# gabo99cas/minimal_volumetric_path_tracer

Hardware: AMD Instinct MI355X
Metric: Msamples/s (pixels×spp/s) at 1024²; per-channel RMSE vs CPU PPM (higher is better)
Workload: dtype f64; 1 GPU; ff 1024x1024x256spp default scene, sigma_a 0.001 sigma_s 0.009; width=1024, height=1024, spp=256, estimator=ff, parallelism=1 GPU, inflight=3

## Files before the change

minimal_volumetric_path_tracer_amd/csrc/vpt_device.h:

```cpp
#ifndef VPT_DEVICE_H
#define VPT_DEVICE_H

#include <hip/hip_runtime.h>
#include <stdint.h>

#include "vpt_math.h"
#include "vpt_rng.h"
#include "vpt_scene.h"

#define VPT_DEV __device__ static inline __attribute__((always_inline))
#define VPT_PI 3.14159265358979323846
#define VPT_MAXFLOAT ((double)3.40282346638528859812e+38F)
#define VPT_DBL_MAX 1.7976931348623157e+308
#ifndef VPT_ISECT_UNROLL
#define VPT_ISECT_UNROLL 5
#endif
#ifndef VPT_DECIDE_GROUP
#define VPT_DECIDE_GROUP 5
#endif
static_assert(VPT_DECIDE_GROUP >= 1, "spheres are taken G >= 1 at a time");

namespace vpt {

#define VPT_UNLIKELY(c) __builtin_expect(!!(c), 0)
#define VPT_LIKELY(c) __builtin_expect(!!(c), 1)

#define ISECT_SQRT(x) vm_sqrt(x)
#ifndef VPT_ISECT_CLASS
#define VPT_ISECT_CLASS 1
#endif

#ifndef VPT_SECTIONS
#define VPT_SECTIONS 0
#endif
enum {
    SECT_SCHED = 0, SECT_LOAD, SECT_S_PLIGHT, SECT_S_MIS, SECT_S_MIS_ISECT, SECT_S_BDSF, SECT_M_SS, SECT_M_SS_DIR,
    SECT_M_SS_ISECT, SECT_M_SS_SHADOW, SECT_M_PHASE, SECT_CONT, SECT_A_PREP, SECT_A_DECIDE, SECT_A_ISECT, SECT_STORE,
    SECT_S_TOTAL, SECT_M_TOTAL, SECT_A_CAMERA, SECT_A_DECIDE_IN, SECT_M_SHADOW_IN, SECT_A_CAMERA_IN, SECT_M_EQA,
    SECT_M_TR, SECT_A_UNIT, SECT_A_R2, SECT_USED,
    SECT_N = 32
};
#if VPT_SECTIONS
static __device__ unsigned long long g_vpt_sect[3 * SECT_N];
__device__ static inline __attribute__((always_inline)) uint32_t* sect_lds()
{
    __shared__ uint32_t a[8][3 * SECT_USED];
    return &a[(threadIdx.x >> 6) & 7][0];
}
#endif
__device__ static inline __attribute__((always_inline)) uint32_t sect_now()
{
#if VPT_SECTIONS
    return (uint32_t)__builtin_amdgcn_s_memtime();
#else
    return 0;
#endif
}
__device__ static inline __attribute__((always_inline)) void sect_add(int k, uint32_t t0)
{
#if VPT_SECTIONS
    const uint32_t dt = sect_now() - t0;
    const unsigned long long act = (unsigned long long)__ballot(1);
    const int first = __ffsll(act) - 1;
    if ((int)(threadIdx.x & 63) == first) {
        uint32_t* a = sect_lds();
        a[k] += dt;
        a[SECT_USED + k] += 1;
        a[2 * SECT_USED + k] += (uint32_t)__popcll(act);
    }
#else
    (void)k;
    (void)t0;
#endif
}
__device__ static inline __attribute__((always_inline)) void sect_init()
{
#if VPT_SECTIONS
    for (int l = threadIdx.x & 63; l < 3 * SECT_USED; l += 64) sect_lds()[l] = 0;
#endif
}
__device__ static inline __attribute__((always_inline)) void sect_flush()
{
#if VPT_SECTIONS
    for (int l = threadIdx.x & 63; l < 3 * SECT_USED; l += 64) {
        const uint32_t v = sect_lds()[l];
        atomicAdd(&g_vpt_sect[l < SECT_USED ? l : l < 2 * SECT_USED ? SECT_N + l - SECT_USED : 2 * SECT_N + l - 2 * SECT_USED],
                  (unsigned long long)v);
    }
#endif
}
#define SECT_BEGIN(name) const uint32_t _sect_##name = sect_now()
#define SECT_END(name, k) sect_add(k, _sect_##name)
// ... 99 lines not shown
            tmin = tact;
            id = i;
        }
    }
}

#ifndef VPT_TAKE_IN
#define VPT_TAKE_IN 1
#endif
#ifndef VPT_ISECT_ZERO
#define VPT_ISECT_ZERO 1
#endif
template <bool ZR = false>
VPT_DEV void sphere_test(double b, double det, int i, double& tmin, int& id, contact_t& contact)
{
    if (!VPT_TAKE_IN) {
        sphere_take(sphere_tact(b, det), i, tmin, id, contact);
        return;
    }
    if (det >= 0) {
        const double sq = (VPT_ISECT_ZERO && ZR) ? vm_sqrt_isect_z(det) : VPT_ISECT_CLASS ? vm_sqrt_isect(det) : ISECT_SQRT(det);
        const double t2 = -b + sq;
        const double t1 = -b - sq;
        sphere_take(t1 < 0.0001 ? t2 : t1, i, tmin, id, contact);
    }
}

template <bool COUNT, bool ZR = false>
VPT_DEV int scene_intersect(const DevScene* __restrict__ S, Sampler<COUNT>& smp, dv3 o, dv3 d, double& t,
                            int& id, bool skip3)
{
    double tmin = VPT_DBL_MAX;
    contact_t contact = 0;
    const int n = S->n;
#pragma unroll VPT_ISECT_UNROLL
    for (int i = 0; i < n; ++i) {
        const GeoSphere g = S->geo[i];
        if (skip3 && g.mat3) continue;
        double ocx = o.x - g.px, ocy = o.y - g.py, ocz = o.z - g.pz;
        double b = ocx * d.x + ocy * d.y + ocz * d.z;
        double cc = ocx * ocx + ocy * ocy + ocz * ocz;
        double det = b * b - cc + g.r2;
        sphere_test<ZR>(b, det, i, tmin, id, contact);
    }
    smp.tests(skip3 ? S->n_non3 : n);
    if (contact) {
        t = tmin;
        return 1;
    }
    t = 0;
    return 0;
}

template <int G, bool COUNT, bool ZR = false>
VPT_DEV int scene_intersect_grouped(const DevScene* __restrict__ S, Sampler<COUNT>& smp, dv3 o, dv3 d, double& t,
                                    int& id)
{
    static_assert(G >= 1, "spheres are taken G >= 1 at a time");
    double tmin = VPT_DBL_MAX;
    contact_t contact = 0;
    const int n = S->n;
    int i = 0;
    for (; i + G <= n; i += G) {
        double b[G], det[G];
#pragma unroll
        for (int k = 0; k < G; ++k) {
            const GeoSphere g = S->geo[i + k];
            const double ocx = o.x - g.px, ocy = o.y - g.py, ocz = o.z - g.pz;
            b[k] = ocx * d.x + ocy * d.y + ocz * d.z;
            const double cc = ocx * ocx + ocy * ocy + ocz * ocz;
            det[k] = b[k] * b[k] - cc + g.r2;
        }
#pragma unroll
        for (int k = 0; k < G; ++k) {
            sphere_test<ZR>(b[k], det[k], i + k, tmin, id, contact);
        }
    }
    for (; i < n; ++i) {
        const GeoSphere g = S->geo[i];
        const double ocx = o.x - g.px, ocy = o.y - g.py, ocz = o.z - g.pz;
        const double b = ocx * d.x + ocy * d.y + ocz * d.z;
        const double cc = ocx * ocx + ocy * ocy + ocz * ocz;
        const double det = b * b - cc + g.r2;
        sphere_test<ZR>(b, det, i, tmin, id, contact);
    }
    smp.tests(n);
    if (contact) {
        t = tmin;
        return 1;
    }
    t = 0;
    return 0;
}

template <int G, bool COUNT, bool ZR = false>
VPT_DEV int scene_intersect_grouped_oc(const DevScene* __restrict__ S, Sampler<COUNT>& smp, const double (*oc)[4],
                                       dv3 d, double& t, int& id)
{
    static_assert(G >= 1, "spheres are taken G >= 1 at a time");
    double tmin = VPT_DBL_MAX;
    contact_t contact = 0;
    const int n = S->n;
    int i = 0;
    for (; i + G <= n; i += G) {
        double b[G], det[G];
#pragma unroll
        for (int k = 0; k < G; ++k) {
            const double ocx = oc[i + k][0], ocy = oc[i + k][1], ocz = oc[i + k][2], cc = oc[i + k][3];
            b[k] = ocx * d.x + ocy * d.y + ocz * d.z;
            det[k] = b[k] * b[k] - cc + S->geo[i + k].r2;
        }
#pragma unroll
        for (int k = 0; k < G; ++k) sphere_test<ZR>(b[k], det[k], i + k, tmin, id, contact);
    }
    for (; i < n; ++i) {
        const double ocx = oc[i][0], ocy = oc[i][1], ocz = oc[i][2], cc = oc[i][3];
        const double b = ocx * d.x + ocy * d.y + ocz * d.z;
        const double det = b * b - cc + S->geo[i].r2;
        sphere_test<ZR>(b, det, i, tmin, id, contact);
    }
    smp.tests(n);
    if (contact) {
        t = tmin;
        return 1;
// ... 1066 lines not shown
    double dist;
    double pdf;
    int id;
    int src;
};

enum { EV_END = 0, EV_SURF = 1, EV_MED = 2 };

VPT_DEV void vpt_opaque(Path& p)
{
    vpt_opaque(p.o);
    vpt_opaque(p.d);
    vpt_opaque(p.beta);
    vpt_opaque(p.L);
    vpt_opaque(p.depth);
}
VPT_DEV void vpt_sink(const Path& p)
{
    vpt_sink(p.o);
    vpt_sink(p.d);
    vpt_sink(p.beta);
    vpt_sink(p.L);
    vpt_sink(p.depth);
}
VPT_DEV void vpt_opaque(Event& e)
{
    vpt_opaque(e.t);
    vpt_opaque(e.dist);
    vpt_opaque(e.pdf);
    vpt_opaque(e.id);
    vpt_opaque(e.src);
}
VPT_DEV void vpt_sink(const Event& e)
{
    vpt_sink(e.t);
    vpt_sink(e.dist);
    vpt_sink(e.pdf);
    vpt_sink(e.id);
    vpt_sink(e.src);
}

template <bool COUNT>
VPT_DEV bool continue_path(Sampler<COUNT>& smp, const Path& p, const Medium& m)
{
    if (m.max_depth > 0 && p.depth >= m.max_depth) return false;
    if (COUNT) smp.cnt.iterations++;
    const double q = 1 - 0.6;
    return !(smp.next() < q);
}

template <int EST>
VPT_DEV constexpr bool est_free_flight() { return EST == 0 || EST == 2 || EST == 3; }

template <int EST, bool COUNT>
VPT_DEV int decide(const DevScene* __restrict__ S, Sampler<COUNT>& smp, Path& p, Event& e, const Medium& m)
{
    const double sigma_t = m.sigma_a + m.sigma_s;
    int id = 0;
    double t = 0.0;
    SECT_BEGIN(di);
#if VPT_DUP == DUP_DECIDE_ISECT
    {
        dv3 o2 = p.o, d2 = p.d;
        vpt_opaque(o2);
        vpt_opaque(d2);
        double t2 = 0;
        int id2 = 0;
        const int h2 = scene_intersect_grouped<VPT_DECIDE_GROUP>(S, smp, o2, d2, t2, id2);
        vpt_sink(t2);
        vpt_sink(id2);
        vpt_sink(h2);
    }
#endif
    const bool hit = scene_intersect_grouped<VPT_DECIDE_GROUP>(S, smp, p.o, p.d, t, id);
    SECT_END(di, SECT_A_ISECT);
    if constexpr (EST == 5) {
        if (COUNT) smp.cnt.iterations++;
        e.t = t;
        e.id = id;
        e.src = 0;
        if (!hit) return EV_END;
        if (S->sph[id].radiance[0] > 0) {
            if (p.depth < 1) p.L = sph_rad(S, id);
            return EV_END;
        }
        return EV_SURF;
    }
    if (!hit) t = VPT_MAXFLOAT;
    e.t = t;
    e.id = id;
    if (EST == 3) {
        const double TrActual = hit ? transmitance(p.o, add(p.o, scl(p.d, t)), sigma_t) : 0.0;
        e.src = 0;
        e.dist = -lm_log(1 - smp.next()) / sigma_t;
        e.pdf = (sigma_t * lm_exp(sigma_t * e.dist * -1.0)) * (1.0 - TrActual);
        if (!(e.dist > t)) return EV_MED;
        if (sph_flag(S->m_emitter, id)) {
            p.L = add(p.L, mul(p.beta, sph_rad(S, id)));
            return EV_END;
        }
        return EV_SURF;
    }
    const int count = S->n_emit;
    if (VPT_UNLIKELY(count == 0)) return EV_END;
    e.src = emit_pick(S, (int)(smp.next() * count), count);
    bool surf;
    if (est_free_flight<EST>()) {
        e.dist = -lm_log(1 - smp.next()) / sigma_t;
        surf = e.dist > t;
    } else {
        const double psurf = EST == 1 ? lm_exp(sigma_t * t * -1.0)
                                      : (hit ? transmitance(p.o, add(p.o, scl(p.d, t)), sigma_t) : 0.0);
        (void)smp.next();
        e.pdf = psurf;
        surf = EST == 1 ? smp.next() < psurf : smp.next() <= psurf;
    }
    if (!surf) return EV_MED;
    if (sph_flag(S->m_emitter, id)) {
        if (p.depth == 0) p.L = EST == 0 ? mul(sph_rad(S, id), p.beta) : sph_rad(S, id);
        return EV_END;
    }
    return EV_SURF;
}

template <int EST, bool COUNT, int MK = -1, int PT = -1>
VPT_DEV void surface_event(const DevScene* __restrict__ S, Sampler<COUNT>& smp, Path& p, const Event& e,
                           const Medium& m, bool cont = true, int lk = -1)
{
    const int ptk = PT >= 0 ? PT : lk;
    const double sigma_t = m.sigma_a + m.sigma_s;
    const double continueprob = 0.6;
    const int id = e.id, src = e.src;
    const dv3 xs = add(p.o, scl(p.d, e.t));
    const dv3 nx = nrm(sub(xs, sph_p(S, id)));
    if (EST == 3) {
        dv3 wi = mk(0, 0, 0);
        double pdf = 0;
        dv3 fs = bdsf<COUNT, MK>(S, smp, wi, p.d, nx, pdf, id);
        wi = nrm(wi);
        const double cosine = dot(nx, wi);
        p.beta = scl(scl(scl(mul(p.beta, fs), (1 / continueprob)), cosine), (1 / pdf));
        p.o = xs;
        p.d = wi;
        p.depth++;
        return;
    }
    const double probSource = 1.0 / S->n_emit;
    const double alpha = S->sph[id].alpha;
    SECT_BEGIN(pl);
    dv3 Ldp = mk(0, 0, 0);
    bool plight_zero = false;
    if (ptk == 0 && S->n_mat3 == 0) {
        const dv3 lx = sub(sph_p(S, src), xs);
        const double dd = dot(lx, lx);
        const double distance = vm_sqrt(dd);
        const bool fin = dd > 0 && dd < VPT_DBL_MAX && nx.x - nx.x == 0 && nx.y - nx.y == 0 && nx.z - nx.z == 0;
        const bool zero = S->sph[src].r > 0.0001 && !(distance < S->sph[src].r) && fin;
        plight_zero = __ballot(!zero) == 0;
        if (plight_zero) smp.tests(2 * S->n);
    }
    Frame Fn = {};
    if (MK == 0 && VPT_FRAME_CSE) Fn = make_frame(nx);
#if VPT_DUP == DUP_PLIGHT
    if (!plight_zero) {
        dv3 xs2 = xs, nx2 = nx, d2 = p.d;
        int id2 = id, src2 = src;
        double a2 = alpha;
        Frame F2 = Fn;
        vpt_opaque(xs2);
        vpt_opaque(nx2);
        vpt_opaque(d2);
// ... 532 lines not shown
```

minimal_volumetric_path_tracer_amd/csrc/vpt_glibm.h:

```cpp
#ifndef VPT_GLIBM_H
#define VPT_GLIBM_H

#if defined(__HIPCC__)
#define GM_TABLE(name, n) __device__ static const double name[n]
#else
#define GM_TABLE(name, n) static const double name[n]
#endif
#include "vpt_glibm_tables.h"

#define GM_UNLIKELY(c) __builtin_expect(!!(c), 0)

VM_QUAL int32_t gm_hi(double x) { return (int32_t)(vm_as_u64(x) >> 32); }
VM_QUAL uint32_t gm_lo(double x) { return (uint32_t)vm_as_u64(x); }
VM_QUAL double gm_fma(double a, double b, double c) { return fma(a, b, c); }
VM_QUAL double gm_fnma(double a, double b, double c) { return fma(-a, b, c); }

VM_TABLE(gm_sc_tab, {
    -0x1.addffc2fcdf59p-26, 0x1.71de27b9a7ed9p-19, -0x1.a01a019db08b8p-13, 0x1.1111111110ecep-7,
    -0x1.5555555555555p-3,
    0x1.11110e829872fp-7, -0x1.5555555555515p-3,
    0x1.6c16bedd9e239p-10, -0x1.5555555555535p-5,
    0x1.8p+45,
    0x1.45f306dc9c883p-1, 0x1.8p52,
    0x1.921fb58000000p+0, -0x1.dde973c000000p-27,
// ... 228 lines not shown
    const double r = gm_fnma(t * t, z, 1.0);
    double q;
    VM_HORNER_T(q, K + GA_RT3, 4, r);
    t = q * t;
    const double c = z * t;
    const double h = gm_fnma(t * 0.5, c, 1.5);
    const double t27 = VM_T(K, GA_T27);
    const double y = gm_fnma(t27, c, gm_fma(c, t27, c));
    const double cc = gm_fnma(y, y, z) / gm_fma(h, c, y);
    double p;
    VM_HORNER_T(p, K + GA_F6, 6, z);
    const double pr = (p * z) * (y + cc);
    const double s = (cc + pr) + y;
    return x == 1.0 ? 0.0 : s + s;
}

VM_TABLE(gm_exp_tab, {
    0x1.71547652b82fep7, 0x1.8p52, -0x1.62e42fefa0000p-8, -0x1.cf79abc9e3b3ap-47,
    0x1.ffffffffffdbdp-2, 0x1.555555555543cp-3, 0x1.55555cf172b91p-5, 0x1.1111167a4d017p-7})
VM_TABLE(gm_log_tab, {
    -0x1.ffffffffffdcbp-3, 0x1.5555555555577p-2, 0x1.24924a344de3p-3, -0x1.55555556745a7p-3,
    -0x1.999eb43b068ffp-4, 0x1.c7184282ad6cap-4, 0x1.999999995dd0cp-3, -0x1.fffffa4423d65p-4,
    0x1.78182f7afd085p-4, -0x1.5521375d145cdp-4, 0x1p27,
    0x1.62e42fefa3800p-1, 0x1.ef35793c76730p-45, -0x1.fffffffeb4590p-3, 0x1.555555551305bp-2,
    -0x1.55575e506c89fp-3, 0x1.999b324f10111p-3, -0x1.0000000000001p-1})
enum { GE_INVLN2N = 0, GE_SHIFT, GE_NLN2HI, GE_NLN2LO, GE_C2, GE_C3, GE_C4, GE_C5 };
enum { GL_B0 = 0, GL_TWO27 = 10, GL_LN2HI, GL_LN2LO, GL_A0, GL_A1, GL_A2, GL_A3, GL_AH };

#define GM_EXP_T(i) gl_tab[(0xAF9D0ull - GL_TAB_LO) / 8 + (i)]
#define GM_LOG_T(i) gl_tab[(0xB0270ull - GL_TAB_LO) / 8 + (i)]

VM_QUAL double gm_exp(double x)
{
    vm_ct* K = vm_tab(gm_exp_tab);
    const uint32_t abstop = (uint32_t)(vm_as_u64(x) >> 52) & 0x7ffu;
    const double z = gm_fma(x, VM_T(K, GE_INVLN2N), VM_T(K, GE_SHIFT));
    const uint64_t ki = vm_as_u64(z);
    const double kd = z - VM_T(K, GE_SHIFT);
    double r = gm_fma(kd, VM_T(K, GE_NLN2HI), x);
    r = gm_fma(kd, VM_T(K, GE_NLN2LO), r);
    const uint32_t idx = 2u * (uint32_t)(ki & 0x7fu);
    const double tail = vm_as_f64(GM_EXP_T(idx));
    const uint64_t sbits = GM_EXP_T(idx + 1) + (ki << 45);
    const double r2 = r * r;
    const double p23 = gm_fma(r, VM_T(K, GE_C3), VM_T(K, GE_C2));
    const double p45 = gm_fma(r, VM_T(K, GE_C5), VM_T(K, GE_C4));
    const double tmp = gm_fma(r2 * r2, p45, gm_fma(p23, r2, r + tail));
    const double scale = vm_as_f64(sbits);
    double v = gm_fma(scale, tmp, scale);
    VM_RARE_FIX(abstop - 0x3c9u >= 0x3fu, v, gl_exp(x));
    return v;
}

VM_QUAL double gm_log(double x)
{
    vm_ct* K = vm_tab(gm_log_tab);
    const uint64_t ix = vm_as_u64(x);
    const uint32_t top = (uint32_t)(ix >> 48);
    const double r1 = x - 1.0;
    const double rr = r1 * r1;
    const double r3 = r1 * rr;
    double a = gm_fma(r1, VM_T(K, GL_B0), VM_T(K, GL_B0 + 1));
    double b = gm_fma(r1, VM_T(K, GL_B0 + 2), VM_T(K, GL_B0 + 3));
    double c = gm_fma(r1, VM_T(K, GL_B0 + 4), VM_T(K, GL_B0 + 5));
    a = gm_fma(rr, VM_T(K, GL_B0 + 6), a);
    b = gm_fma(rr, VM_T(K, GL_B0 + 7), b);
    c = gm_fma(rr, VM_T(K, GL_B0 + 8), c);
    c = gm_fma(r3, VM_T(K, GL_B0 + 9), c);
    c = gm_fma(c, r3, b);
    c = gm_fma(c, r3, a);
    const double two27 = VM_T(K, GL_TWO27);
    const double rhi = gm_fnma(two27, r1, gm_fma(r1, two27, r1));
    const double rhi2 = rhi * rhi;
    const double ah = -0.5;
    const double hi1 = gm_fma(rhi2, ah, r1);
    double lo1 = gm_fma(rhi2, ah, r1 - hi1);
    lo1 = gm_fma(ah * (r1 - rhi), r1 + rhi, lo1);
    double v1 = hi1 + gm_fma(c, r3, lo1);
    v1 = ix == 0x3ff0000000000000ull ? 0.0 : v1;
    const uint64_t tmp = ix + 0xc01a000000000000ull;
    const uint32_t i = (uint32_t)(tmp >> 45) & 0x7fu;
    const int k = (int)((int64_t)tmp >> 52);
    const double zz = vm_as_f64(ix - (tmp & 0xfff0000000000000ull));
    const double kd = (double)k;
    const double invc = vm_as_f64(GM_LOG_T(2 * i)), logc = vm_as_f64(GM_LOG_T(2 * i + 1));
    const double r = gm_fma(zz, invc, -1.0);
    const double w = gm_fma(kd, VM_T(K, GL_LN2HI), logc);
    const double hi = r + w;
    const double r2 = r * r;
    double lo = gm_fma(kd, VM_T(K, GL_LN2LO), (w - hi) + r);
    lo = gm_fma(r2, VM_T(K, GL_AH), lo);
    double q = gm_fma(r, VM_T(K, GL_A2), VM_T(K, GL_A3));
    q = gm_fma(q, r2, gm_fma(r, VM_T(K, GL_A0), VM_T(K, GL_A1)));
    const double v2 = gm_fma(r * r2, q, lo) + hi;
    double v = ix + 0xc012000000000000ull <= 0x308ffffffffffull ? v1 : v2;
    VM_RARE_FIX(top - 0x0010u >= 0x7ff0u - 0x0010u, v, gl_log(x));
    return v;
}

VM_TABLE(gm_atan2_tab, {
    0x1.375f08b31cbcep-4, -0x1.7458022b13c25p-4, 0x1.c71c6e5129a3bp-4, -0x1.24924923f7603p-3,
    0x1.99999999997fdp-3, -0x1.5555555555555p-2,
    0x1.921fb54442d18p+0, 0x1.1a62633145c07p-54,
    0x1p-500, 0x1p500, 0x1p52})
enum { GT_D13 = 0, GT_HPI = 6, GT_HPI1, GT_TM500, GT_T500, GT_TWO52 };
#define GM_CIJ(i, j) vm_as_f64(gl_tab[(0xBE0E0ull - GL_TAB_LO) / 8 + 7 * (i) + (j)])

VM_QUAL double gm_atan2(double y, double x)
{
    vm_ct* K = vm_tab(gm_atan2_tab);
    const double ax = vm_fabs(x), ay = vm_fabs(y);
    const int de = (int)((uint32_t)gm_hi(y) & 0x7ff00000u) - (int)((uint32_t)gm_hi(x) & 0x7ff00000u);
    const int ci = ax > ay;
    const double num = ci ? ay : ax, den = ci ? ax : ay;
    const double u = num / den;
    const double v5 = den * u;
    const double v7 = gm_fma(den, u, -v5);
    const double du = ((num - v5) - v7) / den;
    const double v = u * u;
    double p;
    VM_HORNER_T(p, K + GT_D13, 6, v);
    const double uv = u * v;
    const double hpi = VM_T(K, GT_HPI), hpi1 = VM_T(K, GT_HPI1);
    const double z_i_poly = u + gm_fma(uv, p, du);
    const double t2 = hpi - u;
    const double z_ii_poly = ((((hpi - t2) - u) + hpi1) - du) - uv * p + t2;
    int i = (int)(gm_fma(u, 256.0, VM_T(K, GT_TWO52)) - VM_T(K, GT_TWO52)) - 16;
    i = i < 0 ? 0 : i > 240 ? 240 : i;
    const double c0 = GM_CIJ(i, 0), c1 = GM_CIJ(i, 1), c2 = GM_CIJ(i, 2), c3 = GM_CIJ(i, 3);
    const double c4 = GM_CIJ(i, 4), c5 = GM_CIJ(i, 5), c6 = GM_CIJ(i, 6);
    const double t3 = u - c0;
    const double w = du + t3;
    const double dw = vm_fabs(t3) > vm_fabs(du) ? (t3 - w) + du : (du - w) + t3;
    double q = gm_fma(w, c6, c5);
    q = gm_fma(w, q, c4);
    q = gm_fma(w, q, c3);
    const double z_i_tab = gm_fma(w, c2, gm_fma(dw, c2, (w * w) * q)) + c1;
    const double w2 = t3 + du;
    double q2 = gm_fma(w2, c6, c5);
    q2 = gm_fma(w2, q2, c4);
    q2 = gm_fma(w2, q2, c3);
    q2 = gm_fma(w2, q2, c2);
    const double z_ii_tab = (hpi - c1) + gm_fnma(w2, q2, hpi1);
    const int small = u < 0.0625;
    const double z = ci ? (small ? z_i_poly : z_i_tab) : (small ? z_ii_poly : z_ii_tab);
    double r = vm_copysign(de > 0x38fffff ? hpi : z, y);
    const double tm500 = VM_T(K, GT_TM500), t500 = VM_T(K, GT_T500);
    const int rare = !(x > 0.0) || !(ay > 0.0) || !(x < __builtin_inf()) || !(ay < __builtin_inf()) ||
                     de < -0x38fffff || ax < tm500 || ay < tm500 || ax > t500 || ay > t500;
    VM_RARE_FIX(rare, r, gl_atan2(y, x));
    return r;
// ... 139 lines not shown
```

minimal_volumetric_path_tracer_amd/csrc/vpt_host.cpp:

```cpp
#include <math.h>
#include <stdarg.h>
#include <stdio.h>
#include <stdlib.h>
#include <string.h>

#include <string>
#include <vector>

#include <thread>

#include "vpt_accum.h"
#include "vpt_grid.h"
#include "vpt_internal.h"
#include "vpt_rng.h"

static thread_local std::string g_err;

int vpt_fail(int code, const char* fmt, ...)
{
    char buf[512];
    va_list ap;
    va_start(ap, fmt);
    vsnprintf(buf, sizeof buf, fmt, ap);
    va_end(ap);
    g_err = buf;
    return code;
}

void vpt_clear_error(void) { g_err.clear(); }

int vpt_int_grid_check(const vpt_grid_desc* desc, const float* density, const char* who)
{
    if (!desc || !density) return vpt_fail(VPT_E_INVALID, "%s: NULL grid", who);
    const int32_t n[3] = {desc->nx, desc->ny, desc->nz};
    switch (vpt_grid_bad(n, desc->lo, desc->hi, density)) {
    case 1: return vpt_fail(VPT_E_INVALID, "%s: grid %d x %d x %d (each dimension >= 1, at most 2^27 voxels)", who,
                            desc->nx, desc->ny, desc->nz);
    case 2: return vpt_fail(VPT_E_INVALID, "%s: the box must be finite with hi > lo", who);
    case 3: return vpt_fail(VPT_E_INVALID, "%s: densities must be finite and >= 0", who);
    }
    return VPT_OK;
}

extern "C" {

const char* vpt_last_error(void) { return g_err.c_str(); }
int vpt_abi_version(void) { return VPT_ABI_VERSION; }

uint64_t vpt_stream_state(uint64_t seed, uint64_t pixel_idx, uint64_t sample)
{
    return vpt_stream_start(seed, pixel_idx, sample);
}

void vpt_default_params(vpt_params* p)
{
    if (!p) return;
    memset(p, 0, sizeof *p);
    p->width = 1024;
    p->height = 768;
    p->spp = 16;
    p->fb_format = VPT_FB_F32;
    p->medium.sigma_a = 0.001;
    p->medium.sigma_s = 0.009;
    p->medium.hg_g = 0.0;
    p->medium.max_depth = 0;
    p->medium.estimator = VPT_FREE_FLIGHT;
    p->medium.march_step = 0.1;
    p->medium.march_light = 7;
    p->seed = 0x5EED0001ull;
    double dx = 0, dy = -0.042612, dz = -1;
    double inv = 1.0 / sqrt(dx * dx + dy * dy + dz * dz);
    p->camera.o[0] = 0; p->camera.o[1] = 11.2; p->camera.o[2] = 214;
    p->camera.d[0] = dx * inv; p->camera.d[1] = dy * inv; p->camera.d[2] = dz * inv;
    p->fov_scale = 0.5095;
    p->band_rows = p->height;
    p->band_stride = 1;
    p->band_offset = 0;
}

static void set_sphere(vpt_sphere* s, double r, double px, double py, double pz, double cr, double cg, double cb,
                       double lr, double lg, double lb, int mat, const double* eta, const double* kappa, double alpha)
{
    memset(s, 0, sizeof *s);
    s->r = r;
    s->p[0] = px; s->p[1] = py; s->p[2] = pz;
    s->c[0] = cr; s->c[1] = cg; s->c[2] = cb;
    s->radiance[0] = lr; s->radiance[1] = lg; s->radiance[2] = lb;
    s->material = mat;
    if (eta) memcpy(s->eta, eta, sizeof s->eta);
    if (kappa) memcpy(s->kappa, kappa, sizeof s->kappa);
    s->alpha = alpha;
}

int vpt_default_scene(vpt_sphere* out, int cap)
{
    vpt_sphere s[10];
    static const double al_eta[3] = {1.66058, 0.88143, 0.521467};
// ... 239 lines not shown
```

minimal_volumetric_path_tracer_amd/csrc/vpt_internal.h:

```cpp
#ifndef VPT_INTERNAL_H
#define VPT_INTERNAL_H

#include "../../include/vpt.h"

int vpt_fail(int code, const char* fmt, ...);
void vpt_clear_error(void);

int vpt_int_device(const vpt_context* ctx);
const unsigned* vpt_int_guard_flag(const vpt_context* ctx);
int vpt_int_check_guard(vpt_context* ctx, const char* who);
int vpt_int_check_params(const vpt_context* ctx, const vpt_params* p);
int vpt_int_pool_pass(vpt_context* ctx, const vpt_params* p, int C, int k0, int k1, const unsigned* d_tiles,
                      unsigned n_tiles, double* d_partials, unsigned* d_queue);

int vpt_int_grid_check(const vpt_grid_desc* desc, const float* density, const char* who);

#endif
```

minimal_volumetric_path_tracer_amd/csrc/vpt_kernels.hip:

```cpp
#include <hip/hip_runtime.h>

#include <math.h>
#include <stdlib.h>
#include <string.h>

#include <memory>
#include <mutex>
#include <vector>

#include "vpt_device.h"
#include "vpt_pool.h"
#include "vpt_wave.h"
#include "vpt_internal.h"

#ifndef VPT_MIS_TU
#define VPT_MIS_TU 1
#endif
#if VPT_MIS_TU
namespace vpt {
extern template __global__ void pool_kernel<1, false>(PoolParams P0, Medium m0, const DevScene* __restrict__ S,
                                                      unsigned long long* counters, unsigned long long* stats);
extern template __global__ void pool_kernel<1, false, true>(PoolParams P0, Medium m0, const DevScene* __restrict__ S,
                                                            unsigned long long* counters, unsigned long long* stats);
}
// ... 73 lines not shown
    x_new[3 * i + 1] = xn.y;
    x_new[3 * i + 2] = xn.z;
    idsource[i] = id;
    out_states[i] = smp.X;
}

__global__ void math_probe_kernel(int fn, const double* x, const double* y, double* out, int n)
{
    int i = blockIdx.x * blockDim.x + threadIdx.x;
    if (i >= n) return;
    double a = x[i], b = y[i], r = 0;
    switch (fn) {
    case 0: r = vm_sqrt(a); break;
    case 1: r = lm_exp(a); break;
    case 2: r = lm_log(a); break;
    case 3: r = lm_sin(a); break;
    case 4: r = lm_cos(a); break;
    case 5: r = lm_tan(a); break;
    case 6: r = lm_atan(a); break;
    case 7: r = lm_acos(a); break;
    case 8: r = lm_atan2(a, b); break;
    case 12: r = vm_inv_sqrt(a); break;
    case 10:
    case 11: {
        double sv, cv;
        lm_sincos_acos(a, &sv, &cv);
        r = fn == 10 ? sv : cv;
        break;
    }
    case 14:
    case 15:
    case 16:
    case 17: {
        double q[4];
        lm_dir_trig(a, b, &q[0], &q[1], &q[2], &q[3]);
        r = q[fn - 14];
        break;
    }
    case 18: {
        double bb = b;
        __asm__ volatile("" : "+v"(bb));
        r = vm_div_by(a, vm_rcp_of(bb));
        break;
    }
    case 19: r = hemi_cosine_prob(a); break;
    case 20: {
        double inv, q;
        inv_and_ratio(a, b, inv, q);
        r = __longlong_as_double(__double_as_longlong(inv) ^ __double_as_longlong(q));
        break;
    }
    case 21: r = vm_sqrt_isect(a); break;
    case 22: r = vm_sqrt_isect_z(a); break;
    default: r = a / b; break;
    }
    out[i] = r;
}

__global__ void phase_probe_kernel(double g, double dx, double dy, double dz, const uint64_t* X, int n, double* dirs,
                                   uint64_t* Xout, const double* wl, int nw, double* vals)
{
    const int i = blockIdx.x * blockDim.x + threadIdx.x;
    const dv3 din = mk(dx, dy, dz);
    if (i < n) {
        Sampler<false> smp;
        smp.X = X[i];
        smp.g = g;
        smp.cnt.tests = smp.cnt.iterations = smp.cnt.draw_mismatch = 0;
        const dv3 w = phase_sample(smp, din);
        dirs[3 * i] = w.x;
        dirs[3 * i + 1] = w.y;
        dirs[3 * i + 2] = w.z;
        Xout[i] = smp.X;
    }
    if (i < nw) vals[i] = phase_value(g, din, mk(wl[3 * i], wl[3 * i + 1], wl[3 * i + 2]));
}

bool is_finite(double v) { return v == v && v - v == 0.0; }

unsigned long long* g_pool_stats = nullptr;

}

struct StreamSlot {
    hipStream_t stream;
    unsigned* d_queue;
    double* d_partials;
    size_t partials_bytes;
    hipEvent_t done;
    unsigned long long used;
};
constexpr int MAX_STREAM_SLOTS = 8;
constexpr int LAUNCH_LOG2_MAX = 26;

struct vpt_context {
    int device;
    DevScene* d_scene;
    DevScene h_scene;
    int has_scene;
    unsigned long long* d_counters;
    unsigned* d_guard;
    unsigned guard_bias = 0;
    std::mutex mu;
    std::vector<std::unique_ptr<StreamSlot>> slots;
    unsigned long long tick = 0;
    int launch_log2 = LAUNCH_LOG2_MAX;
// ... 226 lines not shown
        }
        return VPT_OK;
    }
}

static int pool_plan(const KParams& K, vpt_chunk_layout lay, int c0, int c1, const unsigned* tile_map, unsigned n_tiles,
                     PoolParams& Q, uint64_t* first, uint64_t* count)
{
    if (K.w > 65535 || K.h > 65535) return vpt_fail(VPT_E_INVALID, "width and height must be < 65536");
    Q.w = K.w;
    Q.h = K.h;
    Q.spp = K.spp;
    Q.rows = K.shard_rows;
    Q.band_rows = K.band_rows;
    Q.band_stride = K.band_stride;
    Q.band_offset = K.band_offset;
    Q.tiles_x = K.tiles_x;
    Q.lay = lay;
    Q.nch = Q.lay.n;
    Q.level_units = n_tiles * 64u;
    Q.sh_lu = log2_exact((int64_t)Q.level_units);
    Q.sh_tx = log2_exact(K.tiles_x);
    Q.sh_br = log2_exact(K.band_rows);
    Q.sh_bs = log2_exact(K.band_stride);
    Q.sh_c = log2_exact(Q.lay.C);
    Q.rw = log2_exact(K.w) >= 0 ? 1.0 / K.w : 0.0;
    Q.rh = log2_exact(K.h) >= 0 ? 1.0 / K.h : 0.0;
    Q.tile_map = tile_map;
    const uint64_t end = (uint64_t)n_tiles * 64u * (uint64_t)c1;
    if (end >= 0xFFFFFFFFull) return vpt_fail(VPT_E_INVALID, "too many work units (%llu)", (unsigned long long)end);
    *first = (uint64_t)n_tiles * 64u * (uint64_t)c0;
    *count = end - *first;
    Q.seed = K.seed;
    for (int i = 0; i < 3; ++i) {
        Q.o[i] = K.o[i];
        Q.d[i] = K.d[i];
        Q.cx[i] = K.cx[i];
        Q.cy[i] = K.cy[i];
    }
    return VPT_OK;
}

template <int EST>
static int pool_enqueue(vpt_context* ctx, const KParams& K, PoolParams& Q, uint64_t first, uint64_t units, double* partials,
                        unsigned* queue, hipStream_t stream)
{
    const DevScene* S = ctx->d_scene;
    constexpr bool COUNT = false;
    int blocks = 0;
    Q.partials = partials;
    Q.queue = queue;
    Q.guard = ctx->d_guard;
    Q.guard_bias = ctx->guard_bias;
    const Medium m = medium_of(K);
    constexpr bool HAS_TILES = EST <= 1;
    const bool tiles = Q.tile_map != nullptr;
    if (tiles && !HAS_TILES)
        return vpt_fail(VPT_E_UNSUPPORTED, "estimator %d renders whole tile sets only (tile subsets: estimators 0 and 1)", EST);
    int rc;
    if constexpr (HAS_TILES) {
        rc = tiles ? persistent_grid(ctx, pool_kernel<EST, COUNT, true>, &blocks, VPT_POOL_THREADS)
                   : persistent_grid(ctx, pool_kernel<EST, COUNT>, &blocks, VPT_POOL_THREADS);
    } else {
        rc = persistent_grid(ctx, pool_kernel<EST, COUNT>, &blocks, VPT_POOL_THREADS);
    }
    if (rc) return rc;
    const uint64_t need = (units + POOL - 1) / POOL;
    if ((uint64_t)blocks > need) blocks = (int)need;
    if (first + units + (uint64_t)blocks * (UREFILL + 1) >= 0xFFFFFFFFull)
        return vpt_fail(VPT_E_INVALID, "too many work units (%llu) for the u32 work queue", (unsigned long long)(first + units));
    if (Q.lay.C > (1 << LAUNCH_LOG2_MAX))
        return vpt_fail(VPT_E_INVALID, "chunk of %d samples > 2^26 (the per-workgroup launch bound)", Q.lay.C);
    const uint64_t max_units = launch_max_units(blocks, Q.lay.C, ctx->launch_log2);
    unsigned long long* stats = nullptr;
    if (env_int("VPT_POOL_STATS", 0)) {
        if (!g_pool_stats) HIP_OK(hipMalloc((void**)&g_pool_stats, (TL0 + 3 * TL_MAXWG) * sizeof(unsigned long long)));
        HIP_OK(hipMemsetAsync(g_pool_stats, 0, TL0 * sizeof(unsigned long long), stream));
        HIP_OK(hipMemsetAsync(g_pool_stats + TL0, 0xFF, 3 * TL_MAXWG * sizeof(unsigned long long), stream));
        stats = g_pool_stats;
    }
    for (uint64_t u0 = 0; u0 < units; u0 += max_units) {
        Q.unit0 = (unsigned)(first + u0);
        Q.nunits = (unsigned)(units - u0 < max_units ? units - u0 : max_units);
        HIP_OK(hipMemsetAsync(Q.queue, 0, sizeof(unsigned), stream));
        if constexpr (HAS_TILES) {
            if (tiles) pool_kernel<EST, COUNT, true><<<dim3((unsigned)blocks), dim3(VPT_POOL_THREADS), 0, stream>>>(Q, m, S, K.counters, stats);
            else pool_kernel<EST, COUNT><<<dim3((unsigned)blocks), dim3(VPT_POOL_THREADS), 0, stream>>>(Q, m, S, K.counters, stats);
        } else {
            pool_kernel<EST, COUNT><<<dim3((unsigned)blocks), dim3(VPT_POOL_THREADS), 0, stream>>>(Q, m, S, K.counters, stats);
        }
        HIP_OK(hipGetLastError());
    }
    return VPT_OK;
}

template <int EST, int FB>
static int launch_pool(vpt_context* ctx, KParams K, hipStream_t stream)
{
    [[maybe_unused]] constexpr bool COUNT = false;
    int rc;
    const bool wave = EST <= 1 && env_int("VPT_WAVE_KERNEL", 0);
    if (!wave) {
        PoolParams Q;
        uint64_t first = 0, units = 0;
        const vpt_chunk_layout lay = vpt_chunks(K.spp, K.chunk, K.taper);
        rc = pool_plan(K, lay, 0, lay.n, nullptr, (unsigned)K.tiles_x * (unsigned)K.tiles_y, Q, &first, &units);
// ... 775 lines not shown
```

minimal_volumetric_path_tracer_amd/csrc/vpt_pool.h:

```cpp
#ifndef VPT_POOL_H
#define VPT_POOL_H

#include "vpt_chunks.h"
#include "vpt_device.h"

namespace vpt {

#ifndef VPT_POOL_DEBUG
#define VPT_POOL_DEBUG 0
#endif
#ifndef VPT_POOL_THREADS
#define VPT_POOL_THREADS 512
#endif
#ifndef VPT_POOL_WGS
#define VPT_POOL_WGS 1
#endif
#ifndef VPT_KILL_RINGS
#define VPT_KILL_RINGS 1
#endif
#ifndef VPT_SCHED_PRIO
#define VPT_SCHED_PRIO 3
#endif
#ifndef VPT_PREP_TRIES
#define VPT_PREP_TRIES 3
// ... 26 lines not shown
constexpr int NSTATS = 24;
constexpr int TL0 = 32, TL_MAXWG = 4096;
__device__ __forceinline__ void dbg_tl(unsigned long long* stats, int k, bool inv)
{
    const unsigned long long t = __builtin_amdgcn_s_memrealtime();
    if (blockIdx.x < (unsigned)TL_MAXWG) atomicMin(&stats[TL0 + 3 * blockIdx.x + k], inv ? ~t : t);
}
struct ADbg {
    unsigned long long rounds, samples, c_prep, c_decide;
};
__device__ __forceinline__ unsigned long long dbg_clock(bool dbg) { return dbg ? __builtin_amdgcn_s_memtime() : 0; }

enum { F_OX = 0, F_OY, F_OZ, F_DX, F_DY, F_DZ, F_BX, F_BY, F_BZ, F_LX, F_LY, F_LZ, F_AX, F_AY, F_AZ, F_TD, F_KEY,
       F_PDF };

struct TaskPool {
    double2 f2[NF / 2][POOL];
    uint64_t X[POOL];
    uint4 w[POOL];
    uint16_t ring[NR][POOL];
    int ctl[NCTL];
    uint32_t uring[URING];
};

constexpr int SLOT_BITS = POOL > 512 ? 10 : 9, SLOT_MASK = (1 << SLOT_BITS) - 1, LAP_MASK = (1 << (16 - SLOT_BITS)) - 1;
static_assert(POOL <= (1 << SLOT_BITS), "slot ids must fit the ring entry");
__device__ __forceinline__ uint16_t ring_entry(int slot, int pos)
{
    return (uint16_t)(slot | (((pos / POOL) & LAP_MASK) << SLOT_BITS));
}

__device__ __forceinline__ int lds_peek(const int* p)
{
    return __hip_atomic_load(p, __ATOMIC_RELAXED, __HIP_MEMORY_SCOPE_WORKGROUP);
}

struct PoolParams {
    int w, h, spp, rows;
    int band_rows, band_stride, band_offset;
    int tiles_x, nch;
    vpt_chunk_layout lay;
    unsigned level_units;
    unsigned nunits;
    unsigned unit0;
    uint64_t seed;
    double o[3], d[3], cx[3], cy[3];
    int sh_lu, sh_tx, sh_br, sh_bs, sh_c;
    double rw, rh;
    double* partials;
    unsigned* queue;
    unsigned* guard;
    unsigned guard_bias;
    const unsigned* tile_map;
};

#ifndef VPT_P_KARG
#define VPT_P_KARG 1
#endif
#if VPT_P_KARG && defined(__HIP_DEVICE_COMPILE__)
typedef const __attribute__((address_space(4))) PoolParams PoolParamsK;
__device__ __forceinline__ PoolParamsK& pool_params_at_use()
{
    uint64_t a = (uint64_t)(uintptr_t)__builtin_amdgcn_kernarg_segment_ptr();
    __asm__ volatile("" : "+s"(a));
    return *(PoolParamsK*)a;
}
#define VPT_PARAMS(Pin) PoolParamsK& P = pool_params_at_use(); (void)(Pin)
#else
#define VPT_PARAMS(Pin) const PoolParams& P = (Pin)
#endif

template <class LAY>
__device__ __forceinline__ int vpt_chunk_of_end_lay(const LAY& lay, int c1)
{
    const vpt_chunk_layout l = lay;
    return vpt_chunk_of_end(&l, c1);
}
template <class LAY>
__device__ __forceinline__ void vpt_chunk_range_lay(const LAY& lay, int c, int* s0, int* s1)
{
    const vpt_chunk_layout l = lay;
    vpt_chunk_range(&l, c, s0, s1);
}

__device__ __forceinline__ unsigned udiv_p(unsigned a, unsigned d, int sh) { return sh >= 0 ? a >> sh : a / d; }

struct Unit {
    int x, y, c;
    bool valid;
};

template <bool TMAP>
__device__ __forceinline__ Unit decode_unit(const PoolParams& P0, unsigned u)
{
    VPT_PARAMS(P0);
    u += P.unit0;
    Unit r;
    const unsigned c = udiv_p(u, P.level_units, P.sh_lu), rem = u - c * P.level_units;
    r.c = (int)c;
    const unsigned tile = TMAP ? P.tile_map[rem >> 6] : rem >> 6, p = rem & 63u;
    const unsigned ty = udiv_p(tile, (unsigned)P.tiles_x, P.sh_tx);
    r.x = (int)(tile - ty * (unsigned)P.tiles_x) * 8 + (int)(p & 7u);
    const int lr = (int)ty * 8 + (int)(p >> 3);
    r.valid = r.x < P.w && lr < P.rows;
    const int k = (int)udiv_p((unsigned)lr, (unsigned)P.band_rows, P.sh_br), rr = lr - k * P.band_rows;
    const int fr = (P.band_offset + k * P.band_stride) * P.band_rows + rr;
    r.y = P.h - 1 - fr;
// ... 244 lines not shown
            break;
        }
    }
    if (round >= 2) sect_add(SECT_A_R2, t_r2);
    SECT_END(pr, SECT_A_PREP);
    SECT_BEGIN(cam);
    if (fresh) {
        SECT_BEGIN(ci);
        smp.X = t.X;
        const double jx = smp.next();
        const double jy = smp.next();
        if (EST != 5) (void)smp.next();
        t.p.o = mk(P.o[0], P.o[1], P.o[2]);
#if VPT_DUP == DUP_CAMERA
        {
            double jx2 = jx, jy2 = jy;
            int px = (int)(t.pix & 0xFFFFu), py = (int)(t.pix >> 16);
            vpt_opaque(jx2);
            vpt_opaque(jy2);
            vpt_opaque(px);
            vpt_opaque(py);
            vpt_sink(pool_camera_dir(P0, jx2, jy2, px, py));
        }
#endif
        t.p.d = pool_camera_dir(P0, jx, jy, (int)(t.pix & 0xFFFFu), (int)(t.pix >> 16));
        t.p.beta = mk(1, 1, 1);
        t.p.L = mk(0, 0, 0);
        t.p.depth = 0;
        if (EST == 5) t.e.pdf = 1;
        t.X = smp.X;
        SECT_END(ci, SECT_A_CAMERA_IN);
    }
    SECT_END(cam, SECT_A_CAMERA);
    const unsigned long long c1 = dbg_clock(dbg);
    int result = parked ? R_A : R_DONE;
    SECT_BEGIN(dc);
    if (!done && !parked) {
        SECT_BEGIN(dci);
        smp.X = t.X;
#if VPT_DUP == DUP_DECIDE
        {
            Path p2 = t.p;
            Event e2 = t.e;
            vpt_opaque(p2);
            vpt_opaque(e2);
            Sampler<COUNT> s2 = smp;
            vpt_opaque(s2.X);
            vpt_sink(decide<EST>(S, s2, p2, e2, m));
            vpt_sink(p2);
            vpt_sink(e2);
            vpt_sink(s2.X);
        }
#endif
        const int ev = decide<EST>(S, smp, t.p, t.e, m);
        t.X = smp.X;
        if (ev == EV_END) {
            t.acc = add(t.p.L, t.acc);
            t.in_path = false;
            result = R_A;
        } else if (ev == EV_SURF) {
            const int sk = sph_flag(S->m_skey1, t.e.id) | (sph_flag(S->m_skey2, t.e.id) << 1);
            result = R_S + (sk == 0 ? (EST == 3 || EST == 5 ? 0 : sph_flag(S->m_point, t.e.src)) : sk);
            if (kill_predicted_est<EST>() && !COUNT && sk == 0 &&
                path_ends_after_event(t.X, t.p.depth, m, S->kp_sa, S->kp_sc))
                result += R_SD - R_S;
        } else {
            result = R_M + (EST == 3 ? 0 : sph_flag(S->m_point, t.e.src));
            if (!(EST == 1 || EST == 4)) t.e.t = t.e.dist;
            if constexpr (kill_predicted_est<EST>() && !COUNT) {
                uint64_t ja, jc;
                vpt_erand48_jump(5, &ja, &jc);
                if (path_ends_after_event(t.X, t.p.depth, m, ja, jc)) result += R_MD - R_M;
            }
        }
        SECT_END(dci, SECT_A_DECIDE_IN);
    }
    SECT_END(dc, SECT_A_DECIDE);
    if (dbg) {
        D.c_prep += c1 - c0;
        D.c_decide += dbg_clock(dbg) - c1;
    }
    return result;
}

template <int EST, bool COUNT, bool TMAP = false>
__global__ __launch_bounds__(VPT_POOL_THREADS, VPT_POOL_WGS) void pool_kernel(PoolParams P0, Medium m0, const DevScene* __restrict__ S,
                                                   unsigned long long* counters, unsigned long long* stats)
{
    __shared__ TaskPool sh;
#if VPT_P_KARG && defined(__HIP_DEVICE_COMPILE__)
    if (pool_params_at_use().nunits != P0.nunits + P0.guard_bias || pool_params_at_use().unit0 != P0.unit0) {
        if (threadIdx.x == 0) atomicOr(P0.guard, 1u);
        return;
    }
#endif
    const int tid = threadIdx.x, lane = tid & 63;
    const uint64_t below = (1ull << lane) - 1ull;
    for (int j = tid; j < POOL; j += VPT_POOL_THREADS) {
        sh.w[j] = uint4{0u, 0u, 0u, 0u};
        sh.ring[R_A][j] = (uint16_t)j;
        for (int r = 1; r < NR; ++r) sh.ring[r][j] = (uint16_t)(LAP_MASK << SLOT_BITS);
    }
    if (tid < NCTL) sh.ctl[tid] = tid == C_TAIL + R_A ? POOL : 0;
    sect_init();
    __syncthreads();

    Sampler<COUNT> smp;
    smp.X = 0;
    smp.g = m0.g;
    smp.cnt.tests = 0;
    smp.cnt.iterations = 0;
    smp.cnt.draw_mismatch = 0;
    int n = 0, slot = 0, next = R_A;
    unsigned long long st_idle = 0, st_retry = 0, st_sched = 0, st_b[NR] = {}, st_l[NR] = {}, st_c[3] = {};
    ADbg D = {};
    const bool dbg = VPT_POOL_DEBUG && stats != nullptr;
    const bool dbga = VPT_POOL_DEBUG == 1 && dbg;
    unsigned long long tclk = dbg_clock(dbg);
    bool seen_exh = false;
    if (dbg && tid == 0) dbg_tl(stats, 0, false);
    while (true) {
        SECT_BEGIN(sc);
        if (VPT_SCHED_PRIO) __builtin_amdgcn_s_setprio(VPT_SCHED_PRIO);
        if (n > 0) {
            const bool ret = lane < n && next < NR;
            int pos = 0;
            if (ret) pos = __hip_atomic_fetch_add(&sh.ctl[C_TAIL + next], 1, __ATOMIC_RELAXED, __HIP_MEMORY_SCOPE_WORKGROUP);
// ... 228 lines not shown
```

Baseline: 7351 Msamples/s.

## Precompute camera-origin sphere offsets in kernargs and hoist emitter pick/log lookup

Adds a per-launch table of camera-origin-to-sphere offsets and squared distances, filled on the host and passed in the kernel arguments. When every lane in a wave holds a fresh camera ray, the intersection loop reads these values instead of recomputing them. For the free-flight estimators it also draws the emitter pick and log-table lookup before intersection so their latency can overlap the intersection work, and it pins scene bitmasks in scalar registers. This costs a much larger kernarg block (guarded by a 4 KB static_assert) and an extra wave ballot, and whether the camera path triggers depends on how often whole waves are fresh.

```diff
diff --git a/minimal_volumetric_path_tracer_amd/csrc/vpt_device.h b/minimal_volumetric_path_tracer_amd/csrc/vpt_device.h
--- a/minimal_volumetric_path_tracer_amd/csrc/vpt_device.h
+++ b/minimal_volumetric_path_tracer_amd/csrc/vpt_device.h
@@ -37,7 +37,7 @@
     SECT_SCHED = 0, SECT_LOAD, SECT_S_PLIGHT, SECT_S_MIS, SECT_S_MIS_ISECT, SECT_S_BDSF, SECT_M_SS, SECT_M_SS_DIR,
     SECT_M_SS_ISECT, SECT_M_SS_SHADOW, SECT_M_PHASE, SECT_CONT, SECT_A_PREP, SECT_A_DECIDE, SECT_A_ISECT, SECT_STORE,
     SECT_S_TOTAL, SECT_M_TOTAL, SECT_A_CAMERA, SECT_A_DECIDE_IN, SECT_M_SHADOW_IN, SECT_A_CAMERA_IN, SECT_M_EQA,
-    SECT_M_TR, SECT_A_UNIT, SECT_A_R2, SECT_USED,
+    SECT_M_TR, SECT_A_UNIT, SECT_A_R2, SECT_A_PICK, SECT_A_LOG, SECT_A_CLASS, SECT_A_ALLFRESH, SECT_USED,
     SECT_N = 32
 };
 #if VPT_SECTIONS
@@ -243,9 +243,9 @@
     return 0;
 }
 
-template <int G, bool COUNT, bool ZR = false>
+template <int G, bool COUNT, bool ZR = false, class TAB = const double (*)[4]>
 VPT_DEV int scene_intersect_grouped(const DevScene* __restrict__ S, Sampler<COUNT>& smp, dv3 o, dv3 d, double& t,
-                                    int& id)
+                                    int& id, bool cam = false, TAB cam_oc = nullptr)
 {
     static_assert(G >= 1, "spheres are taken G >= 1 at a time");
     double tmin = VPT_DBL_MAX;
@@ -254,13 +254,22 @@
     int i = 0;
     for (; i + G <= n; i += G) {
         double b[G], det[G];
+        if (cam) {
 #pragma unroll
-        for (int k = 0; k < G; ++k) {
-            const GeoSphere g = S->geo[i + k];
-            const double ocx = o.x - g.px, ocy = o.y - g.py, ocz = o.z - g.pz;
-            b[k] = ocx * d.x + ocy * d.y + ocz * d.z;
-            const double cc = ocx * ocx + ocy * ocy + ocz * ocz;
-            det[k] = b[k] * b[k] - cc + g.r2;
+            for (int k = 0; k < G; ++k) {
+                const double ocx = cam_oc[i + k][0], ocy = cam_oc[i + k][1], ocz = cam_oc[i + k][2], cc = cam_oc[i + k][3];
+                b[k] = ocx * d.x + ocy * d.y + ocz * d.z;
+                det[k] = b[k] * b[k] - cc + S->geo[i + k].r2;
+            }
+        } else {
+#pragma unroll
+            for (int k = 0; k < G; ++k) {
+                const GeoSphere g = S->geo[i + k];
+                const double ocx = o.x - g.px, ocy = o.y - g.py, ocz = o.z - g.pz;
+                b[k] = ocx * d.x + ocy * d.y + ocz * d.z;
+                const double cc = ocx * ocx + ocy * ocy + ocz * ocz;
+                det[k] = b[k] * b[k] - cc + g.r2;
+            }
         }
 #pragma unroll
         for (int k = 0; k < G; ++k) {
@@ -1433,12 +1442,25 @@
 template <int EST>
 VPT_DEV constexpr bool est_free_flight() { return EST == 0 || EST == 2 || EST == 3; }
 
-template <int EST, bool COUNT>
-VPT_DEV int decide(const DevScene* __restrict__ S, Sampler<COUNT>& smp, Path& p, Event& e, const Medium& m)
-{
+template <int EST, bool COUNT, bool HOIST = false, class TAB = const double (*)[4]>
+VPT_DEV int decide(const DevScene* __restrict__ S, Sampler<COUNT>& smp, Path& p, Event& e, const Medium& m,
+                   bool cam = false, TAB cam_oc = nullptr, uint64_t m_emitter = 0)
+{
+    constexpr bool hoist = HOIST && (EST == 0 || EST == 2);
     const double sigma_t = m.sigma_a + m.sigma_s;
     int id = 0;
     double t = 0.0;
+    int h_count = 0, h_src = 0;
+    double h_x = 0;
+    gm_log_pair h_lp = {0, 0};
+    if constexpr (hoist) {
+        h_count = S->n_emit;
+        if (VPT_LIKELY(h_count != 0)) {
+            h_src = emit_pick(S, (int)(smp.next() * h_count), h_count);
+            h_x = 1 - smp.next();
+            h_lp = gm_log_pair_of(h_x);
+        }
+    }
     SECT_BEGIN(di);
 #if VPT_DUP == DUP_DECIDE_ISECT
     {
@@ -1453,7 +1475,7 @@
         vpt_sink(h2);
     }
 #endif
-    const bool hit = scene_intersect_grouped<VPT_DECIDE_GROUP>(S, smp, p.o, p.d, t, id);
+    const bool hit = scene_intersect_grouped<VPT_DECIDE_GROUP>(S, smp, p.o, p.d, t, id, cam, cam_oc);
     SECT_END(di, SECT_A_ISECT);
     if constexpr (EST == 5) {
         if (COUNT) smp.cnt.iterations++;
@@ -1482,12 +1504,18 @@
         }
         return EV_SURF;
     }
-    const int count = S->n_emit;
+    SECT_BEGIN(pk);
+    const int count = hoist ? h_count : S->n_emit;
     if (VPT_UNLIKELY(count == 0)) return EV_END;
-    e.src = emit_pick(S, (int)(smp.next() * count), count);
+    if constexpr (hoist) e.src = h_src;
+    else e.src = emit_pick(S, (int)(smp.next() * count), count);
+    SECT_END(pk, SECT_A_PICK);
     bool surf;
     if (est_free_flight<EST>()) {
-        e.dist = -lm_log(1 - smp.next()) / sigma_t;
+        SECT_BEGIN(lg);
+        if constexpr (hoist) e.dist = -gm_log_finish(h_x, h_lp) / sigma_t;
+        else e.dist = -lm_log(1 - smp.next()) / sigma_t;
+        SECT_END(lg, SECT_A_LOG);
         surf = e.dist > t;
     } else {
         const double psurf = EST == 1 ? lm_exp(sigma_t * t * -1.0)
@@ -1497,7 +1525,7 @@
         surf = EST == 1 ? smp.next() < psurf : smp.next() <= psurf;
     }
     if (!surf) return EV_MED;
-    if (sph_flag(S->m_emitter, id)) {
+    if (sph_flag(hoist ? m_emitter : S->m_emitter, id)) {
         if (p.depth == 0) p.L = EST == 0 ? mul(sph_rad(S, id), p.beta) : sph_rad(S, id);
         return EV_END;
     }
diff --git a/minimal_volumetric_path_tracer_amd/csrc/vpt_glibm.h b/minimal_volumetric_path_tracer_amd/csrc/vpt_glibm.h
--- a/minimal_volumetric_path_tracer_amd/csrc/vpt_glibm.h
+++ b/minimal_volumetric_path_tracer_amd/csrc/vpt_glibm.h
@@ -304,7 +304,21 @@
     return v;
 }
 
-VM_QUAL double gm_log(double x)
+typedef struct {
+    double invc, logc;
+} gm_log_pair;
+
+VM_QUAL gm_log_pair gm_log_pair_of(double x)
+{
+    const uint64_t tmp = vm_as_u64(x) + 0xc01a000000000000ull;
+    const uint32_t i = (uint32_t)(tmp >> 45) & 0x7fu;
+    gm_log_pair t;
+    t.invc = vm_as_f64(GM_LOG_T(2 * i));
+    t.logc = vm_as_f64(GM_LOG_T(2 * i + 1));
+    return t;
+}
+
+VM_QUAL double gm_log_finish(double x, gm_log_pair t)
 {
     vm_ct* K = vm_tab(gm_log_tab);
     const uint64_t ix = vm_as_u64(x);
@@ -331,11 +345,10 @@
     double v1 = hi1 + gm_fma(c, r3, lo1);
     v1 = ix == 0x3ff0000000000000ull ? 0.0 : v1;
     const uint64_t tmp = ix + 0xc01a000000000000ull;
-    const uint32_t i = (uint32_t)(tmp >> 45) & 0x7fu;
     const int k = (int)((int64_t)tmp >> 52);
     const double zz = vm_as_f64(ix - (tmp & 0xfff0000000000000ull));
     const double kd = (double)k;
-    const double invc = vm_as_f64(GM_LOG_T(2 * i)), logc = vm_as_f64(GM_LOG_T(2 * i + 1));
+    const double invc = t.invc, logc = t.logc;
     const double r = gm_fma(zz, invc, -1.0);
     const double w = gm_fma(kd, VM_T(K, GL_LN2HI), logc);
     const double hi = r + w;
@@ -349,6 +362,8 @@
     VM_RARE_FIX(top - 0x0010u >= 0x7ff0u - 0x0010u, v, gl_log(x));
     return v;
 }
+
+VM_QUAL double gm_log(double x) { return gm_log_finish(x, gm_log_pair_of(x)); }
 
 VM_TABLE(gm_atan2_tab, {
     0x1.375f08b31cbcep-4, -0x1.7458022b13c25p-4, 0x1.c71c6e5129a3bp-4, -0x1.24924923f7603p-3,
diff --git a/minimal_volumetric_path_tracer_amd/csrc/vpt_host.cpp b/minimal_volumetric_path_tracer_amd/csrc/vpt_host.cpp
--- a/minimal_volumetric_path_tracer_amd/csrc/vpt_host.cpp
+++ b/minimal_volumetric_path_tracer_amd/csrc/vpt_host.cpp
@@ -42,7 +42,25 @@
     return VPT_OK;
 }
 
+void vpt_int_cam_table(const double* o, const double* centre, size_t stride, int n, double (*oc)[4])
+{
+    for (int i = 0; i < n; ++i, centre += stride) {
+        const double ocx = o[0] - centre[0], ocy = o[1] - centre[1], ocz = o[2] - centre[2];
+        oc[i][0] = ocx;
+        oc[i][1] = ocy;
+        oc[i][2] = ocz;
+        oc[i][3] = ocx * ocx + ocy * ocy + ocz * ocz;
+    }
+}
+
 extern "C" {
+
+int vpt_debug_cam_table(const vpt_sphere* spheres, int n, const double* o, double* out)
+{
+    if (!spheres || !o || !out || n < 0 || n > VPT_MAX_SPHERES) return vpt_fail(VPT_E_INVALID, "vpt_debug_cam_table: bad arguments");
+    vpt_int_cam_table(o, spheres[0].p, sizeof(vpt_sphere) / sizeof(double), n, (double (*)[4])out);
+    return VPT_OK;
+}
 
 const char* vpt_last_error(void) { return g_err.c_str(); }
 int vpt_abi_version(void) { return VPT_ABI_VERSION; }
diff --git a/minimal_volumetric_path_tracer_amd/csrc/vpt_internal.h b/minimal_volumetric_path_tracer_amd/csrc/vpt_internal.h
--- a/minimal_volumetric_path_tracer_amd/csrc/vpt_internal.h
+++ b/minimal_volumetric_path_tracer_amd/csrc/vpt_internal.h
@@ -1,5 +1,7 @@
 #ifndef VPT_INTERNAL_H
 #define VPT_INTERNAL_H
+
+#include <stddef.h>
 
 #include "../../include/vpt.h"
 
@@ -13,6 +15,8 @@
 int vpt_int_pool_pass(vpt_context* ctx, const vpt_params* p, int C, int k0, int k1, const unsigned* d_tiles,
                       unsigned n_tiles, double* d_partials, unsigned* d_queue);
 
+void vpt_int_cam_table(const double* o, const double* centre, size_t stride, int n, double (*oc)[4]);
+
 int vpt_int_grid_check(const vpt_grid_desc* desc, const float* density, const char* who);
 
 #endif
diff --git a/minimal_volumetric_path_tracer_amd/csrc/vpt_kernels.hip b/minimal_volumetric_path_tracer_amd/csrc/vpt_kernels.hip
--- a/minimal_volumetric_path_tracer_amd/csrc/vpt_kernels.hip
+++ b/minimal_volumetric_path_tracer_amd/csrc/vpt_kernels.hip
@@ -149,6 +149,13 @@
     }
     case 21: r = vm_sqrt_isect(a); break;
     case 22: r = vm_sqrt_isect_z(a); break;
+    case 23: {
+        gm_log_pair lp = gm_log_pair_of(a);
+        vpt_opaque(lp.invc);
+        vpt_opaque(lp.logc);
+        r = gm_log_finish(a, lp);
+        break;
+    }
     default: r = a / b; break;
     }
     out[i] = r;
@@ -481,6 +488,8 @@
     Q.queue = queue;
     Q.guard = ctx->d_guard;
     Q.guard_bias = ctx->guard_bias;
+    memset(Q.cam_oc, 0, sizeof Q.cam_oc);
+    vpt_int_cam_table(K.o, &ctx->h_scene.geo[0].px, sizeof(GeoSphere) / sizeof(double), ctx->h_scene.n, Q.cam_oc);
     const Medium m = medium_of(K);
     constexpr bool HAS_TILES = EST <= 1;
     const bool tiles = Q.tile_map != nullptr;
diff --git a/minimal_volumetric_path_tracer_amd/csrc/vpt_pool.h b/minimal_volumetric_path_tracer_amd/csrc/vpt_pool.h
--- a/minimal_volumetric_path_tracer_amd/csrc/vpt_pool.h
+++ b/minimal_volumetric_path_tracer_amd/csrc/vpt_pool.h
@@ -102,7 +102,9 @@
     unsigned* guard;
     unsigned guard_bias;
     const unsigned* tile_map;
+    double cam_oc[VPT_MAX_SPHERES][4];
 };
+static_assert(sizeof(PoolParams) + sizeof(Medium) + 3 * sizeof(void*) <= 4096, "pool_kernel's arguments: at most 4 KB");
 
 #ifndef VPT_P_KARG
 #define VPT_P_KARG 1
@@ -453,27 +455,42 @@
             vpt_sink(s2.X);
         }
 #endif
-        const int ev = decide<EST>(S, smp, t.p, t.e, m);
+        constexpr bool CAM = kill_predicted_est<EST>() && !COUNT;
+        const bool cam = CAM && __ballot(!fresh) == 0;
+#if VPT_SECTIONS
+        if (__ballot(!fresh) == 0) sect_add(SECT_A_ALLFRESH, sect_now());
+#endif
+        constexpr bool HOIST = EST == 0 || EST == 2;
+        uint64_t w_emitter = 0, w_point = 0, w_skey1 = 0, w_skey2 = 0, w_kpa = 0, w_kpc = 0;
+        if constexpr (HOIST) {
+            w_emitter = S->m_emitter, w_point = S->m_point, w_skey1 = S->m_skey1, w_skey2 = S->m_skey2;
+            w_kpa = S->kp_sa, w_kpc = S->kp_sc;
+            __asm__ volatile("" : "+s"(w_emitter), "+s"(w_point), "+s"(w_skey1), "+s"(w_skey2), "+s"(w_kpa), "+s"(w_kpc));
+        }
+        const int ev = decide<EST, COUNT, true>(S, smp, t.p, t.e, m, cam, P.cam_oc, w_emitter);
+        SECT_BEGIN(cl);
         t.X = smp.X;
         if (ev == EV_END) {
             t.acc = add(t.p.L, t.acc);
             t.in_path = false;
             result = R_A;
         } else if (ev == EV_SURF) {
-            const int sk = sph_flag(S->m_skey1, t.e.id) | (sph_flag(S->m_skey2, t.e.id) << 1);
-            result = R_S + (sk == 0 ? (EST == 3 || EST == 5 ? 0 : sph_flag(S->m_point, t.e.src)) : sk);
+            const int sk = sph_flag(HOIST ? w_skey1 : S->m_skey1, t.e.id) | (sph_flag(HOIST ? w_skey2 : S->m_skey2, t.e.id) << 1);
+            result = R_S + (sk == 0 ? (EST == 3 || EST == 5 ? 0 : sph_flag(HOIST ? w_point : S->m_point, t.e.src)) : sk);
             if (kill_predicted_est<EST>() && !COUNT && sk == 0 &&
-                path_ends_after_event(t.X, t.p.depth, m, S->kp_sa, S->kp_sc))
+                path_ends_after_event(t.X, t.p.depth, m, HOIST ? w_kpa : S->kp_sa, HOIST ? w_kpc : S->kp_sc))
                 result += R_SD - R_S;
         } else {
-            result = R_M + (EST == 3 ? 0 : sph_flag(S->m_point, t.e.src));
+            result = R_M + (EST == 3 ? 0 : sph_flag(HOIST ? w_point : S->m_point, t.e.src));
             if (!(EST == 1 || EST == 4)) t.e.t = t.e.dist;
             if constexpr (kill_predicted_est<EST>() && !COUNT) {
                 uint64_t ja, jc;
                 vpt_erand48_jump(5, &ja, &jc);
+                if constexpr (HOIST) __asm__ volatile("" : "+s"(ja), "+s"(jc));
                 if (path_ends_after_event(t.X, t.p.depth, m, ja, jc)) result += R_MD - R_M;
             }
         }
+        SECT_END(cl, SECT_A_CLASS);
         SECT_END(dci, SECT_A_DECIDE_IN);
     }
     SECT_END(dc, SECT_A_DECIDE);
```

Result: faster. 7430 Msamples/s, median of 6 (+1.1%).
